# holandes22/etcd

Measured on AMD Instinct MI355X. Metric: MsgAppResp applied/sec + commits advanced/sec, 1M raft groups×3, 1-8 GPUs, higher is better.
Workload: dtype u64

## Files before the change

etcd_amd/csrc/hipbatch.hip:

```cpp
#include <hip/hip_runtime.h>

#include <algorithm>
#include <cstdio>
#include <cstdlib>
#include <cstring>
#include <type_traits>
#include <utility>
#include <vector>

#include "hbmem.h"
#include "hipbatch_kernels.h"
#include "hipbatch_fast.h"
#include "hipbatch_elect.h"
#include "hipbatch_lead.h"
#include "hipbatch_wire.h"
#include "hipbatch_wire_in.h"
#include "hipbatch_wire_out.h"
#include "hipbatch_bin.h"

using namespace hb;

#define HB_CHECK(expr)                                                       \
  do {                                                                       \
    hipError_t _e = (expr);                                                  \
// ... 1067 lines not shown
  for (uint32_t i = tid; i < RG; i += ROUTE_THREADS) {
    const uint32_t c = l_cnt[i], g = gbase + i;
    bool hand = false, elect = false, ok = true;
    if (g < G) {
      bool hib = false;
      uint64_t meta = 0;
      if (EL && c > 0) meta = a.S.meta[g];
      if (hi_on && c <= (uint32_t)KMAX) {
        const uint64_t t = a.S.term[g];
#pragma unroll
        for (uint32_t k = 0; k < (uint32_t)KMAX; ++k) {
          if (k < c) {
            const uint4 r = l_slot[k][i];
            uint64_t tm, ix;
            rec_unpack(r.x, r.y, (uint64_t)r.z | ((uint64_t)r.w << 32), a.side, &tm, &ix);
            hib |= tm > t;
          }
        }
      }
      a.cnt[g] = (uint8_t)((c < CNT_MASK ? c : CNT_MASK) | (hib ? CNT_HIGHER : 0u));
      if constexpr (EL) {
        if (c > 0) {
          const uint32_t cls = handover_class((uint32_t)meta, c, hib, a.nmax, (uint32_t)KMAX);
          elect = cls == HO_ELECT;
          hand = elect || cls == HO_APPLY;
          ok = hand || cls == HO_NONE;
          if (hand) a.resume[g] = 1u << 30;
        }
        e_c = c;
        e_hand = hand;
        e_elect = elect;
        e_meta = meta;
      } else {
#pragma unroll
        for (uint32_t k = 0; k < (uint32_t)KMAX; ++k) {
          if (k < c) {
            at32(a.slot, k * G + g) = l_slot[k][i];
            if constexpr (X) at32(a.slotx, k * G + g) = l_slotx[k][i];
          }
        }
      }
    }
    uint32_t s = c;
#pragma unroll
    for (int d = 32; d >= 1; d >>= 1) s += __shfl_xor(s, d);
    if ((tid & 63) == 0 && s) atomicAdd(&l_ptot[i >> PART_LOG], s);
    if constexpr (EL) {
      const uint64_t b = __ballot(hand), bad = __ballot(!ok);
      if ((tid & 63) == 0) {
        l_pf[i >> 5] = (uint32_t)b;
        l_pf[(i >> 5) + 1] = (uint32_t)(b >> 32);
        if (bad) atomicAnd(&l_ok[i >> PART_LOG], 0u);
      }
    }
  }
  __syncthreads();
  if (tid < NP) {
    const uint32_t part = (bk << sl) + w * NP + tid;
    if (part < a.NB) {
      const uint32_t r = atomicAdd(&a.bk_fill[bk * CTR_STRIDE], a.ev_per_msg * (l_ptot[tid] + PART * a.props_on));
      const uint64_t mo =
          (uint64_t)a.ev_per_msg * ((uint64_t)a.NB * PART + lo + ((uint64_t)bk * PART << sl) * a.props_on) + r;
      a.ev_off[2 * part + 1] = mo;
      if constexpr (EL) l_moff[tid] = mo;
    }
  }
  if constexpr (EL) {
    __syncthreads();
    const uint32_t p = __builtin_amdgcn_readfirstlane(tid >> PART_LOG);
    const uint32_t g = gbase + tid;
    const bool closed = l_ok[p] != 0;
    bool done = false;
    uint32_t st_msgs = 0, st_app = 0, st_vote = 0, st_drop = 0, st_commit = 0;
    ElectLane<EN> L;
    L.won = L.lost = L.nev = 0;
    L.committed = L.last = 0;
    uint64_t last0 = 0;
    if (closed) {
      L.S = a.S;
      L.E.chunk = a.ev + l_moff[p];
      L.E.fill = &l_efill[p];
      L.g = g;
      L.meta = e_meta;
      const bool mine = e_elect && e_c <= (uint32_t)KMAX && L.self() < L.n() && !(L.meta & M_NC);
      if (mine) {
        L.load();
        last0 = L.last;
        const uint64_t commit0 = L.committed;
        uint32_t key[KMAX];
#pragma unroll
        for (uint32_t k = 0; k < (uint32_t)KMAX; ++k) key[k] = k < e_c ? l_slot[k][tid].y : 0xFFFFFFFFu;
        const uint32_t perm = arrival_perm<(uint32_t)KMAX>(key);
        uint32_t x = 0;
#pragma nounroll
        for (; x < e_c; ++x) {
          uint32_t inf, org;
          uint64_t mterm, ix;
          slot_unpack(l_slot[(perm >> (4 * x)) & 0xF][tid], a.side, &inf, &org, &mterm, &ix);
          const uint32_t type = inf & 0xF, from = (inf >> 4) & 0xF;
          if (from >= L.n() && is_response(type)) {
            st_drop++;
            continue;
          }
          if (!L.takes(type, from, mterm)) break;
          L.step(type, from, mterm, (inf >> 8) & 1u);
          st_msgs++;
          st_app += type == HB_MSG_APP_RESP;
          st_vote += type == HB_MSG_VOTE_RESP;
        }
        if (x > 0) {
          L.store();
          if (x == e_c) {
            done = true;
          } else {
            a.resume[g] = x;
            a.commit0[g] = commit0;
          }
        }
        st_commit = done && L.committed != commit0;
      }
      flag_put<false>(&l_pf[p * FLAG_WORDS], tid & (PART - 1), done);
    }
    if (g < G && e_c > 0 && (!closed || (e_hand && !done))) {
#pragma unroll
      for (uint32_t k = 0; k < (uint32_t)KMAX; ++k)
        if (k < e_c) at32(a.slot, k * G + g) = l_slot[k][tid];
    }
    const uint32_t vals[ST_N + 1] = {st_msgs, st_app, st_vote, st_drop, st_commit, L.won, L.lost, 0,
                                     (uint32_t)(L.last - last0), L.nev};
    reduce_stats(a, l_stats, vals);
    if (tid < NP * FLAG_WORDS) {
      const uint32_t p = tid / FLAG_WORDS, j = tid % FLAG_WORDS, part = (bk << sl) + w * NP + p;
      if (part < a.NB && l_ok[p]) a.pflag[(size_t)part * FLAG_WORDS + j] = l_pf[p * FLAG_WORDS + j];
    }
    if (tid < NP) {
      const uint32_t part = (bk << sl) + w * NP + tid;
      if (part < a.NB) {
        a.lskip[part] = (uint8_t)l_ok[tid];
        if (l_ok[tid]) {
          a.ev_off[2 * part] = (uint64_t)part * PART * a.ev_per_msg;
          a.ev_counts[2 * part] = 0;
          a.ev_counts[2 * part + 1] = l_efill[tid];
          uint32_t any = 0;
#pragma unroll
          for (uint32_t j = 0; j < FLAG_WORDS; ++j) any |= l_pf[tid * FLAG_WORDS + j];
          const uint32_t xs = blockIdx.x & 7;
          if (any) a.ap_list[(size_t)xs * a.NB + atomicAdd(&a.ap_cnt[xs * CTR_STRIDE], 1u)] = part;
        }
      }
    }
  }
}

template <int NMAX, uint32_t KS, bool STEADY = false>
__device__ __forceinline__ bool fast_step(const ApplyArgs& a, FollowLane<NMAX>& L, uint32_t part, uint32_t lane,
                                          bool live, bool lead, bool leader, bool fol, uint32_t prop_raw, uint32_t cnt,
                                          uint32_t (&s_info)[KS], uint32_t (&s_orig)[KS],
                                          uint64_t (&s_term)[KS], uint64_t (&s_index)[KS],
                                          uint64_t (&s_h)[KS], uint64_t (&s_c)[KS],
                                          uint64_t moff, uint32_t* l_pfill, uint32_t* l_fill, uint32_t* l_flag,
                                          uint32_t* l_eflag, uint32_t (&vals)[ST_N + 1], uint32_t& nsteady) {
  constexpr uint32_t KMAX = KS;
  const uint32_t g = part * PART + lane;
  const uint64_t last0 = L.last, commit0 = L.committed;

  bool flagged = false;
  uint32_t resume = 0;
  uint32_t st_msgs = 0, st_drop = 0, st_app = 0;

  const uint64_t poff = (uint64_t)part * PART * a.ev_per_msg;
  if (lane == 0) a.ev_off[2 * part] = poff;
  const uint32_t prop_k = live ? prop_raw : 0u;
  if constexpr (STEADY) {
    static_assert(NMAX == 3 && KS == 2, "SteadyLane is the n = 3, two-slot lane");
    if (a.steady) {
      const bool work = live && (prop_k != 0 || cnt != 0);
      const bool idle = !work && (!lead || (!(L.mlo & (uint32_t)M_RS) && L.self() < 3));
      SteadyLane P;
      P.ok = false;
      P.evm = 0;
      if (lead && work) P.plan(L, prop_k, cnt, s_info, s_orig, s_term, s_index);
      const bool steady = lead && work && P.ok;
      if (__ballot(!(steady || idle)) == 0) {
        const uint32_t evm = steady ? P.evm : 0u;
        uint32_t tot = 0, base = 0;
#pragma unroll
        for (uint32_t j = 0; j < SteadyLane::EW_P; ++j) tot += (uint32_t)__popcll(__ballot((evm >> j) & 1u));
        if (tot && (lane & 63) == 0) base = atomicAdd(l_pfill, tot);
        base = __builtin_amdgcn_readfirstlane(base);
        uint64_t* chunk = a.ev + poff;
#pragma unroll
        for (uint32_t j = 0; j < SteadyLane::EW_P; ++j) {
          const uint64_t m = __ballot((evm >> j) & 1u);
          if ((evm >> j) & 1u) chunk[base + mbcnt64(m)] = P.word(j, lane);
          base += (uint32_t)__popcll(m);
        }
        tot = 0;
        base = 0;
#pragma unroll
        for (uint32_t j = SteadyLane::EW_P; j < SteadyLane::EW; ++j) tot += (uint32_t)__popcll(__ballot((evm >> j) & 1u));
        if (tot && (lane & 63) == 0) base = atomicAdd(l_fill, tot);
        base = __builtin_amdgcn_readfirstlane(base);
        chunk = a.ev + moff;
#pragma unroll
        for (uint32_t j = SteadyLane::EW_P; j < SteadyLane::EW; ++j) {
          const uint64_t m = __ballot((evm >> j) & 1u);
          if ((evm >> j) & 1u) chunk[base + mbcnt64(m)] = P.word(j, lane);
          base += (uint32_t)__popcll(m);
        }
        if (steady) P.commit(L);
        vals[ST_MSGS] = steady ? cnt : 0u;
        vals[ST_APPRESP] = steady ? cnt : 0u;
        vals[ST_VOTERESP] = 0;
        vals[ST_DROPPED] = 0;
        vals[ST_COMMITS] = (uint32_t)(steady && P.committed != commit0);
        vals[ST_WON] = 0;
        vals[ST_LOST] = 0;
        vals[ST_FAULTS] = 0;
        vals[ST_ENTRIES] = steady ? (uint32_t)(P.last - last0) : 0u;
        vals[ST_N] = steady ? P.nev() : 0u;
        if (a.steady_cnt && __ballot(g < a.S.G) != 0) ++nsteady;
        return false;
      }
    }
  }
  L.E.chunk = a.ev + poff;
  L.E.fill = l_pfill;
  if (prop_k) {
    if (lead && L.prop_ok(prop_k)) {
      L.arrival = 0xFFFFFFFFu;
      L.prop(prop_k);
    } else {
      flagged = true;
      resume = 1u << 31;
    }
  }

#pragma unroll
  for (uint32_t k = 0; k < KMAX; ++k) s_orig[k] = k < cnt ? s_orig[k] : 0xFFFFFFFFu;
#pragma unroll
  for (uint32_t r = 0; r < KMAX; ++r) {
#pragma unroll
    for (uint32_t k = (r & 1); k + 1 < KMAX; k += 2) {
      const bool sw = s_orig[k + 1] < s_orig[k];
      const uint32_t i0 = s_info[k], o0 = s_orig[k];
      const uint64_t t0 = s_term[k], x0 = s_index[k], h0 = s_h[k], c0 = s_c[k];
      s_info[k] = sw ? s_info[k + 1] : i0;
      s_orig[k] = sw ? s_orig[k + 1] : o0;
      s_term[k] = sw ? s_term[k + 1] : t0;
      s_index[k] = sw ? s_index[k + 1] : x0;
      s_h[k] = sw ? s_h[k + 1] : h0;
      s_c[k] = sw ? s_c[k + 1] : c0;
      s_info[k + 1] = sw ? i0 : s_info[k + 1];
      s_orig[k + 1] = sw ? o0 : s_orig[k + 1];
      s_term[k + 1] = sw ? t0 : s_term[k + 1];
      s_index[k + 1] = sw ? x0 : s_index[k + 1];
      s_h[k + 1] = sw ? h0 : s_h[k + 1];
      s_c[k + 1] = sw ? c0 : s_c[k + 1];
    }
  }
  L.E.chunk = a.ev + moff;
  L.E.fill = l_fill;
  uint32_t j = 0;
  if (live && !lead && !fol && cnt > 0 && !flagged) {
    flagged = true;
    resume = 0;
  }
  if (live && cnt > KMAX && !flagged && !L.faulted()) {
    flagged = true;
    resume = 0;
  }
  if (lead) {
#pragma unroll
    for (uint32_t k = 0; k < KMAX; ++k) {
      if (k >= cnt || flagged || L.faulted()) break;
      const uint32_t inf = s_info[k];
      const uint32_t type = inf & 0xF, from = (inf >> 4) & 0xF;
      const bool reject = (inf >> 8) & 1u;
      if (from >= L.n() && is_response(type)) {
        st_drop++;
        j++;
        continue;
      }
      if (KMAX >= 3 && type == HB_MSG_PROP) {
        if (s_term[k] != 0 || s_index[k] > 0xFFFFFFFFull || !L.prop_ok((uint32_t)s_index[k])) {
          flagged = true;
          resume = j;
          break;
        }
        L.arrival = s_orig[k];
        L.prop((uint32_t)s_index[k]);
        st_msgs++;
        j++;
        continue;
      }
      if (!L.accept_ok(type, from, s_term[k], reject)) {
        flagged = true;
        resume = j;
        break;
      }
      L.arrival = s_orig[k];
      L.accept(from, s_index[k]);
      st_msgs++;
      if (KMAX >= 3) st_app++;
      j++;
    }
  }
  bool fstepped = false;
  if (fol) {
#pragma unroll
    for (uint32_t k = 0; k < KMAX; ++k) {
      if (k >= cnt || flagged || L.faulted()) break;
      const uint32_t inf = s_info[k];
      const uint32_t from = (inf >> 4) & 0xF;
      if (!L.takes_follow(inf, from, s_term[k], s_index[k], s_h[k], s_c[k])) {
        flagged = true;
        resume = j;
        break;
      }
      L.arrival = s_orig[k];
      L.step_follow(inf, from, s_term[k], s_index[k], s_h[k], s_c[k]);
      fstepped = true;
      st_msgs++;
      j++;
    }
  }

  if (lead) L.store();
  if (fstepped) L.store_follow();
  const bool stored = lead || fstepped;
  if constexpr (NMAX >= 5) {
    bool higher = false;
#pragma unroll
    for (uint32_t k = 0; k < KMAX; ++k) higher |= k < cnt && s_term[k] > L.term;
    flag_put<true>(l_eflag, lane, flagged && (!leader || higher));
  }
  flag_put<true>(l_flag, lane, flagged);
  if (flagged) {
    at32(a.resume, g) = resume | (stored ? 0u : 1u << 30);
    if (stored) at32(a.commit0, g) = commit0;
  }
  vals[ST_MSGS] = st_msgs;
  vals[ST_APPRESP] = KMAX >= 3 ? st_app : (lead ? st_msgs : 0u);
  vals[ST_VOTERESP] = 0;
  vals[ST_DROPPED] = st_drop;
  vals[ST_COMMITS] = (uint32_t)(!flagged && L.committed != commit0);
  vals[ST_WON] = 0;
  vals[ST_LOST] = 0;
  vals[ST_FAULTS] = (uint32_t)(L.faulted() != 0 && live);
  vals[ST_ENTRIES] = (uint32_t)(L.last - last0);
  vals[ST_N] = L.nev;
  return flagged;
}

__device__ __forceinline__ void fast_close(const ApplyArgs& a, uint32_t part, const uint32_t* l_flag,
                                           const uint32_t* l_eflag, uint32_t pfill, uint32_t fill) {
  a.ev_counts[2 * part] = pfill;
  a.ev_counts[2 * part + 1] = fill;
  uint32_t any = 0, eany = 0;
#pragma unroll
  for (uint32_t w = 0; w < FLAG_WORDS; ++w) {
    any |= l_flag[w];
    eany |= l_eflag ? l_eflag[w] : 0u;
  }
  const uint32_t xs = blockIdx.x & 7;
  if (any)
    a.ap_list[(size_t)xs * a.NB + atomicAdd(&a.ap_cnt[xs * CTR_STRIDE], 1u)] = part;
  if (eany)
    a.el_list[(size_t)xs * a.NB + atomicAdd(&a.el_cnt[xs * CTR_STRIDE], 1u)] = part;
}

template <int NMAX, bool X, uint32_t KMAX>
__global__ void __launch_bounds__(PART, HB_FAST_WAVES) k_apply_fast(ApplyArgs a) {
  static_assert(NMAX <= 3, "n >= 5 leaders and followers step in k_apply_lead");
  __shared__ uint32_t l_fill, l_pfill;
  __shared__ uint32_t l_flag[FLAG_WORDS];
  __shared__ uint32_t l_eflag[FLAG_WORDS];
  __shared__ uint64_t l_stats[ST_N + 1];
  __shared__ uint32_t l_steady;

  const uint32_t part = block_part(a.sis_log);
  if (part >= a.NB) return;
  const uint32_t tid = threadIdx.x;
  const uint32_t g = part * PART + tid;
  const bool gvalid = g < a.S.G;
  if (tid == 0) l_fill = l_pfill = l_steady = 0;
  if (tid <= ST_N) l_stats[tid] = 0;
  if (tid < FLAG_WORDS) l_flag[tid] = l_eflag[tid] = 0;

  FollowLane<NMAX> L;
  L.S = a.S;
  L.g = g;
  L.mlo = gvalid ? at32(reinterpret_cast<uint32_t*>(a.S.meta), 2 * g) : 0u;
  const uint32_t prop_raw = (a.props && gvalid) ? at32(a.props, g) : 0u;
  const uint32_t cnt = gvalid ? at32(a.cnt, g) & CNT_MASK : 0u;
  if (gvalid) L.load_head();
  const bool live = gvalid && L.n() != 0 && L.faulted() == 0;
  const bool leader = live && L.state() == HB_STATE_LEADER;
  const bool nc = (L.mlo & (uint32_t)M_NC) != 0;
  const bool lead = leader && !nc && (cnt <= KMAX || prop_raw != 0);
  const bool fol = X && live && !nc && L.state() == HB_STATE_FOLLOWER && cnt > 0 && cnt <= KMAX && prop_raw == 0;
  L.dirty = 0;
  L.nev = 0;
  if (lead) {
    L.load_rest();
  } else if (fol) {
    L.load_follow();
  } else {
    L.last = L.committed = 0;
    if (!(NMAX >= 5 && leader)) L.term = 0;
  }
  uint32_t s_info[KMAX], s_orig[KMAX];
  uint64_t s_term[KMAX], s_index[KMAX], s_h[KMAX], s_c[KMAX];
  const bool slots = (lead || fol) && cnt <= KMAX;
  uint4 raw[KMAX];
#pragma unroll
  for (uint32_t k = 0; k < KMAX; ++k) {
    const bool u = NMAX >= 5 ? leader && k < cnt : slots && k < cnt;
    raw[k] = u ? at32(a.slot, k * a.S.G + g) : make_uint4(0, 0, 0, 0);
  }
#pragma unroll
  for (uint32_t k = 0; k < KMAX; ++k) slot_unpack(raw[k], a.side, &s_info[k], &s_orig[k], &s_term[k], &s_index[k]);
#pragma unroll
  for (uint32_t k = 0; k < KMAX; ++k) {
    uint4 x = make_uint4(0, 0, 0, 0);
    if (X && fol && k < cnt) x = at32(a.slotx, k * a.S.G + g);
    s_h[k] = (uint64_t)x.x | ((uint64_t)x.y << 32);
    s_c[k] = (uint64_t)x.z | ((uint64_t)x.w << 32);
  }
  uint32_t vals[ST_N + 1];
  constexpr bool STEADY = NMAX == 3 && KMAX == 2 && !X;
  uint32_t nsteady = 0;
  (void)fast_step<NMAX, KMAX, STEADY>(a, L, part, tid, live, lead, leader, fol, prop_raw, cnt, s_info, s_orig, s_term,
                                      s_index, s_h, s_c, a.ev_off[2 * part + 1], &l_pfill, &l_fill, l_flag, l_eflag, vals,
                                      nsteady);
  if (STEADY && a.steady_cnt && nsteady && (tid & 63) == 0) atomicAdd(&l_steady, nsteady);
  reduce_stats(a, l_stats, vals);
  if (STEADY && a.steady_cnt && tid == 0 && l_steady) atomicAdd(a.steady_cnt, l_steady);
  if (tid < FLAG_WORDS) a.pflag[(size_t)part * FLAG_WORDS + tid] = l_flag[tid];
  if constexpr (NMAX >= 5) {
    if (tid < FLAG_WORDS) a.eflag[(size_t)part * FLAG_WORDS + tid] = l_eflag[tid];
  }
  if (tid == 0) fast_close(a, part, l_flag, NMAX >= 5 ? l_eflag : nullptr, l_pfill, l_fill);
}

#ifndef HB_RF_UNROLL
#define HB_RF_UNROLL 4
#endif
#ifndef HB_RF_THREADS
#define HB_RF_THREADS 512
#endif
#ifndef HB_RF_RG_LOG
#define HB_RF_RG_LOG 11
#endif
#ifndef HB_RF_WAVES
#define HB_RF_WAVES 4
#endif
constexpr uint32_t RF_THREADS = HB_RF_THREADS;
constexpr uint32_t RF_UNROLL = HB_RF_UNROLL;
template <uint32_t KMAX, bool X> struct RouteFastGeom {
  static constexpr uint32_t RG_LOG = HB_RF_RG_LOG - (KMAX > 2 ? 1u : 0u) - (X ? 1u : 0u);
  static constexpr uint32_t RG = 1u << RG_LOG;
  static constexpr uint32_t NP = RG / PART;
};
template <uint32_t KMAX, bool X>
__global__ void __launch_bounds__(RF_THREADS, HB_RF_WAVES) k_route_fast(ApplyArgs a) {
  constexpr int NMAX = 3;
  using GM = RouteFastGeom<KMAX, X>;
  constexpr uint32_t RG = GM::RG, NP = GM::NP;
  const uint32_t sl = a.sis_log, W = 1u << (PART_LOG + sl - GM::RG_LOG);
  __shared__ uint32_t l_cnt[RG];
  __shared__ uint4 l_slot[KMAX][RG];
  __shared__ uint4 l_slotx[X ? KMAX : 1][X ? RG : 1];
  __shared__ uint32_t l_ptot[NP];
  __shared__ uint64_t l_moff[NP];
  __shared__ uint32_t l_fill[NP], l_pfill[NP];
  __shared__ uint32_t l_flag[NP][FLAG_WORDS];
  __shared__ uint64_t l_stats[ST_N + 1];
  const uint32_t x = blockIdx.x, q = x >> 3;
  const uint32_t bk = ((q / W) << 3) | (x & 7), w = q % W;
  if (bk >= a.NBK) return;
  const uint32_t tid = threadIdx.x;
  const uint32_t G = a.S.G;
  const uint32_t lg0 = w * RG;
  for (uint32_t i = tid; i < RG; i += RF_THREADS) l_cnt[i] = 0;
  if (tid < NP) {
    l_ptot[tid] = 0;
    l_fill[tid] = l_pfill[tid] = 0;
  }
  for (uint32_t i = tid; i < NP * FLAG_WORDS; i += RF_THREADS) (&l_flag[0][0])[i] = 0;
  if (tid <= ST_N) l_stats[tid] = 0;
  __syncthreads();
  const uint32_t lo = a.bk_off[bk], hi = a.bk_off[bk + 1];
  const uint32_t sub_lo = lg0 >> PART_LOG, sub_hi = (lg0 + RG) >> PART_LOG;
  for (uint32_t base = lo; base < hi; base += RF_THREADS * RF_UNROLL) {
    MsgRec m[RF_UNROLL];
    uint4 mx[X ? RF_UNROLL : 1];
    uint32_t sub[RF_UNROLL];
#pragma unroll
    for (uint32_t u = 0; u < RF_UNROLL; ++u) {
      const uint32_t p = base + u * RF_THREADS + tid;
      if (p < hi) m[u] = a.rec[p];
      if constexpr (X) mx[u] = p < hi ? a.recx[p] : make_uint4(0, 0, 0, 0);
      sub[u] = p < hi ? rec_sub(m[u].info) : 0xFFu;
    }
    if (w == 0) {
#pragma unroll
      for (uint32_t u = 0; u < RF_UNROLL; ++u) {
        const uint32_t p = base + u * RF_THREADS + tid;
        if (p < hi) a.key[p] = (uint8_t)sub[u];
      }
    }
#pragma unroll
    for (uint32_t u = 0; u < RF_UNROLL; ++u) {
      const uint32_t p = base + u * RF_THREADS + tid;
      const bool own = p < hi && sub[u] >= sub_lo && sub[u] < sub_hi;
      const uint32_t l = own ? (((sub[u] - sub_lo) << PART_LOG) | ((m[u].info >> 16) & (PART - 1))) : RG;
      if (l < RG) {
        const uint32_t r = atomicAdd(&l_cnt[l], 1u);
        if (r < KMAX) {
          l_slot[r][l] = make_uint4(m[u].info, m[u].orig, (uint32_t)m[u].ti, (uint32_t)(m[u].ti >> 32));
          if constexpr (X) l_slotx[r][l] = mx[X ? u : 0];
        }
      }
    }
  }
  __syncthreads();
  for (uint32_t i = tid; i < RG; i += RF_THREADS) {
    uint32_t s = l_cnt[i];
#pragma unroll
    for (int d = 32; d >= 1; d >>= 1) s += __shfl_xor(s, d);
    if ((tid & 63) == 0 && s) atomicAdd(&l_ptot[i >> PART_LOG], s);
  }
  __syncthreads();
  const uint32_t part0 = (bk << sl) + w * NP;
  if (tid < NP) {
    const uint32_t part = part0 + tid;
    uint64_t mo = 0;
    if (part < a.NB) {
      const uint32_t r = atomicAdd(&a.bk_fill[bk * CTR_STRIDE], a.ev_per_msg * (l_ptot[tid] + PART * a.props_on));
      mo = (uint64_t)a.ev_per_msg * ((uint64_t)a.NB * PART + lo + ((uint64_t)bk * PART << sl) * a.props_on) + r;
      a.ev_off[2 * part + 1] = mo;
    }
    l_moff[tid] = mo;
    l_ptot[tid] = 0;
  }
  __syncthreads();
  uint32_t acc[ST_N + 1];
#pragma unroll
  for (int k = 0; k <= ST_N; ++k) acc[k] = 0;
  constexpr bool STEADY = KMAX == 2 && !X;
  uint32_t nsteady = 0;
  for (uint32_t i = tid; i < RG; i += RF_THREADS) {
    const uint32_t p = STEADY ? (uint32_t)__builtin_amdgcn_readfirstlane(i >> PART_LOG) : i >> PART_LOG;
    const uint32_t part = part0 + p, lane = i & (PART - 1);
    const uint32_t g = part * PART + lane;
    const bool gvalid = part < a.NB && g < G;
    uint64_t moff = l_moff[p];
    if constexpr (STEADY)
      moff = (uint64_t)(uint32_t)__builtin_amdgcn_readfirstlane((uint32_t)moff) |
             (uint64_t)(uint32_t)__builtin_amdgcn_readfirstlane((uint32_t)(moff >> 32)) << 32;
    FollowLane<NMAX> L;
    L.S = a.S;
    L.g = g;
    L.mlo = gvalid ? at32(reinterpret_cast<uint32_t*>(a.S.meta), 2 * g) : 0u;
    const uint32_t prop_raw = (a.props && gvalid) ? at32(a.props, g) : 0u;
    const uint32_t c = gvalid ? l_cnt[i] : 0u;
    const uint32_t cnt = c < CNT_MASK ? c : CNT_MASK;
    if (gvalid) L.load_head();
    const bool live = gvalid && L.n() != 0 && L.faulted() == 0;
    const bool leader = live && L.state() == HB_STATE_LEADER;
    const bool nc = (L.mlo & (uint32_t)M_NC) != 0;
    const bool lead = leader && !nc && (cnt <= KMAX || prop_raw != 0);
    const bool fol = X && live && !nc && L.state() == HB_STATE_FOLLOWER && cnt > 0 && cnt <= KMAX && prop_raw == 0;
    L.dirty = 0;
    L.nev = 0;
    if (lead) {
      L.load_rest();
    } else if (fol) {
      L.load_follow();
    } else {
      L.last = L.committed = 0;
      L.term = 0;
    }
    uint32_t s_info[KMAX], s_orig[KMAX];
    uint64_t s_term[KMAX], s_index[KMAX], s_h[KMAX], s_c[KMAX];
    const bool slots = (lead || fol) && cnt <= KMAX;
#pragma unroll
    for (uint32_t k = 0; k < KMAX; ++k) {
      const bool u = slots && k < cnt;
      slot_unpack(u ? l_slot[k][i] : make_uint4(0, 0, 0, 0), a.side, &s_info[k], &s_orig[k], &s_term[k], &s_index[k]);
      uint4 xe = make_uint4(0, 0, 0, 0);
      if constexpr (X) {
        if (fol && k < cnt) xe = l_slotx[k][i];
      }
      s_h[k] = (uint64_t)xe.x | ((uint64_t)xe.y << 32);
      s_c[k] = (uint64_t)xe.z | ((uint64_t)xe.w << 32);
    }
    uint32_t vals[ST_N + 1];
    const bool flagged = fast_step<NMAX, KMAX, STEADY>(a, L, part, lane, live, lead, leader, fol, prop_raw, cnt, s_info,
                                                       s_orig, s_term, s_index, s_h, s_c, moff, &l_pfill[p],
                                                       &l_fill[p], l_flag[p], nullptr, vals, nsteady);
#pragma unroll
    for (int k = 0; k <= ST_N; ++k)
      if (!(STEADY && k == ST_APPRESP)) acc[k] += vals[k];
    if (flagged) {
      a.cnt[g] = (uint8_t)cnt;
#pragma unroll
      for (uint32_t k = 0; k < KMAX; ++k) {
        if (k < c) {
          at32(a.slot, k * G + g) = l_slot[k][i];
          if constexpr (X) at32(a.slotx, k * G + g) = l_slotx[k][i];
        }
      }
    }
  }
  if constexpr (STEADY) acc[ST_APPRESP] = acc[ST_MSGS];
  if (STEADY && a.steady_cnt && nsteady && (tid & 63) == 0) atomicAdd(&l_ptot[0], nsteady);
  reduce_stats(a, l_stats, acc);
  if (STEADY && a.steady_cnt && tid == 0 && l_ptot[0]) atomicAdd(a.steady_cnt, l_ptot[0]);
  for (uint32_t j = tid; j < NP * FLAG_WORDS; j += RF_THREADS) {
    const uint32_t p = j / FLAG_WORDS, part = part0 + p;
    if (part < a.NB) a.pflag[(size_t)part * FLAG_WORDS + j % FLAG_WORDS] = l_flag[p][j % FLAG_WORDS];
  }
  if (tid < NP && part0 + tid < a.NB) fast_close(a, part0 + tid, l_flag[tid], nullptr, l_pfill[tid], l_fill[tid]);
}

#ifndef HB_GEN_WAVES
#define HB_GEN_WAVES 2
#endif
struct GenShared {
  Stage<CHUNK> sl;
  uint32_t l_fill;
  uint32_t l_flag[FLAG_WORDS];
  uint32_t l_next[FLAG_WORDS];
  uint64_t l_stats[ST_N + 1];
};

template <int NMAX, bool FOLLOW>
__device__ __forceinline__ bool apply_part(const ApplyArgs& a, uint32_t part, GenShared& sh, bool chained) {
  const uint32_t tid = threadIdx.x;
  const uint32_t bk = part >> a.sis_log, sub = part & ((1u << a.sis_log) - 1);
  const uint32_t g = part * PART + tid;
  const uint32_t fill0 = chained ? sh.l_fill : a.ev_counts[2 * part + 1];
  if (tid < FLAG_WORDS) {
    sh.l_flag[tid] = chained ? sh.l_next[tid] : a.pflag[(size_t)part * FLAG_WORDS + tid];
    sh.l_next[tid] = 0;
  }
  __syncthreads();
  uint32_t any = 0;
#pragma unroll
  for (uint32_t w = 0; w < FLAG_WORDS; ++w) any |= sh.l_flag[w];
  if (!any) return false;
  const bool flagged = (sh.l_flag[tid >> 5] >> (tid & 31)) & 1u;

  if (tid == 0) sh.l_fill = fill0;
  if (tid <= ST_N) sh.l_stats[tid] = 0;

  Lane<NMAX, FOLLOW> L;
  L.S = a.S;
  L.E.chunk = a.ev + a.ev_off[2 * part + 1];
  L.E.fill = &sh.l_fill;
  L.g = g;
  L.won = 0;
  L.lost = 0;
  L.nev = 0;
  L.dirty = 0;
  L.prog = false;
  L.voted = false;
  L.meta = 0;
  L.last = 0;
  L.committed = 0;
  uint32_t resume = 0;
  uint64_t commit0 = 0;
  if (flagged) {
    L.meta = a.S.meta[g];
    L.load_group();
    resume = a.resume[g];
    commit0 = ((resume >> 30) & 1u) ? L.committed : a.commit0[g];
  }
  const uint64_t last0 = L.last;
  uint32_t st_msgs = 0, st_app = 0, st_vote = 0, st_drop = 0;
  const uint32_t skip = resume & 0x3FFFFFFFu;
  uint32_t j = 0;
  bool handed = false;
  uint32_t hand_at = 0;
  const uint32_t lo = a.bk_off[bk], hi = a.bk_off[bk + 1];

  constexpr uint32_t KS = route_kmax(NMAX);
  const uint32_t cnt = flagged ? a.cnt[g] & CNT_MASK : 0u;
  const bool by_slot = flagged && cnt <= a.kmax;
  const bool by_walk = flagged && !by_slot;
  __syncthreads();
  auto step_one = [&](uint32_t inf, uint32_t morig, uint64_t mterm, uint64_t mindex, uint32_t ordinal) -> bool {
    const uint32_t type = inf & 0xF, from = (inf >> 4) & 0xF;
    const bool reject = (inf >> 8) & 1u;
    if (!FOLLOW && is_follower_type(type)) {
      handed = true;
      hand_at = ordinal;
      return false;
    }
    if (from >= L.n() && is_response(type)) {
      st_drop++;
      return true;
    }
    L.arrival = morig;
    L.voted = (inf & HB_INFO_VOTED) != 0;
    const bool wants_hint = (reject && type == HB_MSG_APP_RESP) || (FOLLOW && is_follower_type(type));
    L.step(type, from, mterm, mindex, reject, (wants_hint && a.hint) ? a.hint[morig] : 0ull);
    st_msgs++;
    st_app += type == HB_MSG_APP_RESP;
    st_vote += type == HB_MSG_VOTE_RESP;
    return true;
  };
  if (by_slot) {
    if (resume >> 31) {
      L.arrival = 0xFFFFFFFFu;
      L.step(HB_MSG_PROP, L.self(), 0, a.props[g], false, 0);
    }
    uint32_t key[KS];
    uint32_t perm = 0;
#pragma unroll
    for (uint32_t k = 0; k < KS; ++k) {
      key[k] = k < cnt ? at32(a.slot, k * a.S.G + g).y : 0xFFFFFFFFu;
      perm |= k << (4 * k);
    }
#pragma unroll
    for (uint32_t r = 0; r < KS; ++r) {
#pragma unroll
      for (uint32_t k = (r & 1); k + 1 < KS; k += 2) {
        const uint32_t k0 = key[k], k1 = key[k + 1];
        const bool sw = k1 < k0;
        key[k] = sw ? k1 : k0;
        key[k + 1] = sw ? k0 : k1;
        const uint32_t p0 = (perm >> (4 * k)) & 0xF, p1 = (perm >> (4 * (k + 1))) & 0xF;
        const uint32_t swp = (perm & ~(0xFFu << (4 * k))) | (p1 << (4 * k)) | (p0 << (4 * (k + 1)));
        perm = sw ? swp : perm;
      }
    }
    uint32_t inf_n = 0, orig_n = 0;
    uint64_t term_n = 0, index_n = 0;
    if (cnt > skip)
      slot_unpack(at32(a.slot, ((perm >> (4 * skip)) & 0xF) * a.S.G + g), a.side, &inf_n, &orig_n, &term_n, &index_n);
#pragma nounroll
    for (uint32_t x = skip; x < cnt; ++x) {
      if (L.faulted()) break;
      const uint32_t inf = inf_n, morig = orig_n;
      const uint64_t mterm = term_n, mindex = index_n;
      if (x + 1 < cnt)
        slot_unpack(at32(a.slot, ((perm >> (4 * (x + 1))) & 0xF) * a.S.G + g), a.side, &inf_n, &orig_n, &term_n,
                    &index_n);
      if (!step_one(inf, morig, mterm, mindex, x)) break;
    }
  }

// ... 4159 lines not shown
```

etcd_amd/csrc/hipbatch_fast.h:

```cpp
#pragma once

#include "hipbatch_kernels.h"

namespace hb {

template <int NMAX>
struct FastLane {
  DevState S;
  EvSink E;
  uint32_t g;
  uint32_t arrival;
  uint64_t term, committed, first, last, tfirst, tlast;
  uint32_t mlo;
  uint64_t match[NMAX], next[NMAX], head[NMAX];
  uint32_t pm[NMAX];
  uint32_t dirty;
  uint32_t hv;
  static constexpr bool HEADS = NMAX <= 5;
  uint32_t nev;

  __device__ __forceinline__ uint32_t n() const { return (mlo >> 2) & 7; }
  __device__ __forceinline__ uint32_t state() const { return mlo & 3; }
  __device__ __forceinline__ uint32_t self() const { return (mlo >> 5) & 0xF; }
  __device__ __forceinline__ uint32_t faulted() const { return (mlo >> 17) & 0xF; }
// ... 289 lines not shown

  __device__ __forceinline__ void prop(uint32_t k) {
    const uint64_t old = last;
    if (sz_on(S.max_msg_size))
      sz_append(S, g, old, k, term, S.edesc + (arrival == 0xFFFFFFFFu ? S.peoff[g] : S.eoff[arrival]));
    last += k;
    if (tfirst == HB_NO_INDEX) {
      tfirst = old + 1;
      dirty |= D_TFIRST;
    }
    tlast = last;
    dirty |= D_LAST | D_TRUN;
    ev(HB_EV_LAST, 0, 0, last);
    const uint32_t sf = self();
#pragma unroll
    for (int s = 0; s < NMAX; ++s) {
      if ((uint32_t)s == sf) {
        if (match[s] < last) {
          match[s] = last;
          set_pm(s, pm[s] & ~PM_PAUSED);
        }
        if (next[s] < last + 1) next[s] = last + 1;
        dirty |= 1u << (D_SLOT0 + s);
      }
    }
    maybe_commit();
    bcast_append();
    if (faulted()) ev(HB_EV_FAULT, 0, faulted(), arrival_x());
  }

  __device__ __forceinline__ void accept(uint32_t from, uint64_t index) {
    bool updated = false, old_paused = false;
#pragma unroll
    for (int s = 0; s < NMAX; ++s) {
      if ((uint32_t)s == from) {
        old_paused = pm_count(pm[s]) == S.W;
        const uint64_t nx0 = next[s];
        if (next[s] < index + 1) next[s] = index + 1;
        if (match[s] < index) {
          match[s] = index;
          set_pm(s, pm[s] & ~PM_PAUSED);
          updated = true;
          free_to(s, index, nx0);
        }
        dirty |= 1u << (D_SLOT0 + s);
      }
    }
    if (!updated) return;
    if (maybe_commit()) {
      bcast_append();
    } else if (old_paused && !faulted()) {
#pragma unroll
      for (int s = 0; s < NMAX; ++s)
        if ((uint32_t)s == from) send_append(s);
    }
    if (faulted()) ev(HB_EV_FAULT, 0, faulted(), arrival_x());
  }
};

struct SteadyFol {
  uint64_t match, next;
  uint32_t pm;
};

struct SteadyLane {
  static constexpr uint32_t EW_P = 3, EW = 7;
  static constexpr uint32_t EVM_BCAST = 0x54, EVM_COMMIT = 0x2A;
  uint64_t last, committed, tfirst, tlast;
  uint64_t smatch, snext;
  uint32_t spm;
  SteadyFol fa, fb;
  uint32_t spm0, pa0, pb0;
  uint32_t sf, sa, sb;
  uint32_t evm;
  uint32_t ltm;
  uint32_t jfirst;
  uint64_t xfirst;
  uint32_t ring_a, ring_b;
  bool add_a, add_b, touch_a, touch_b;
  bool prop, d_tfirst;
  bool ok;

  __device__ __forceinline__ uint32_t lt_cur(uint64_t x) const { return (tfirst <= x && x <= tlast) ? 1u : 0u; }

  __device__ __forceinline__ uint64_t send(SteadyFol& f, uint32_t& ring, bool& add, bool& touch, uint32_t W,
                                           uint64_t first) {
    const uint32_t c = pm_count(f.pm);
    ok = ok && c != W && f.next >= first;
    const uint64_t x = f.next - 1;
    if (f.next <= last) {
      uint32_t idx = pm_start(f.pm) + c;
      if (idx >= W) idx -= W;
      ring = idx;
      add = true;
      f.next = last + 1;
      touch = true;
      f.pm = pm_make(HB_PR_REPLICATE, pm_paused(f.pm), pm_start(f.pm), c + 1);
    }
    ok = ok && f.next == last + 1;
    return x;
  }
  __device__ __forceinline__ void bcast(uint32_t W, uint64_t first, uint32_t j) {
    const uint64_t xa = send(fa, ring_a, add_a, touch_a, W, first);
    const uint64_t xb = send(fb, ring_b, add_b, touch_b, W, first);
    ok = ok && xa == xb;
    if (jfirst == 0) {
      jfirst = j;
      xfirst = xa;
    }
    evm |= 1u << j;
    ltm |= lt_cur(xa) << j;
  }
  __device__ __forceinline__ bool maybe_commit(uint64_t term, uint64_t first, uint32_t j) {
    const uint64_t mx = umax64(smatch, fa.match), mn = umin64(smatch, fa.match);
    const uint64_t mci = umax64(mn, umin64(mx, fb.match));
    const bool teq = (mci + 1 < first || mci > last) ? term == 0 : (tfirst <= mci && mci <= tlast);
    const bool up = mci > committed && teq;
    ok = ok && !(up && (last < mci || (evm & EVM_COMMIT) != 0));
    if (up) {
      committed = mci;
      evm |= 1u << j;
    }
    return up;
  }
  __device__ __forceinline__ void ack(uint32_t info, uint64_t mterm, uint64_t index, uint64_t term, uint32_t W,
                                      uint64_t first, uint32_t t) {
    const uint32_t type = info & 0xF, from = (info >> 4) & 0xF;
    const bool reject = (info >> 8) & 1u;
    ok = ok && type == HB_MSG_APP_RESP && !reject && (mterm == 0 || mterm == term) && (from == sa || from == sb);
    const bool isa = from == sa;
    const uint64_t am = fa.match, an = fa.next, bm = fb.match, bn = fb.next;
    const uint32_t ap = fa.pm, bp = fb.pm;
    const uint64_t m0 = isa ? am : bm, nx0 = isa ? an : bn;
    const uint32_t p0 = isa ? ap : bp;
    const uint32_t c = pm_count(p0);
    ok = ok && c != W && m0 < index && index <= last && nx0 != 0 && index >= nx0 - 1;
    const uint64_t nx = umax64(nx0, index + 1);
    uint32_t idx = pm_start(p0) + c;
    if (c != 0 && idx >= W) idx -= W;
    const uint32_t p = pm_make(HB_PR_REPLICATE, 0, idx, 0);
    fa.match = isa ? index : am;
    fa.next = isa ? nx : an;
    fa.pm = isa ? p : ap;
    touch_a = touch_a || isa;
    fb.match = isa ? bm : index;
    fb.next = isa ? bn : nx;
    fb.pm = isa ? bp : p;
    touch_b = touch_b || !isa;
    add_a = add_a && !isa;
    add_b = add_b && isa;
    if (maybe_commit(term, first, EW_P + 2 * t)) bcast(W, first, EW_P + 2 * t + 1);
  }

  __device__ __forceinline__ void plan(const FastLane<3>& L, uint32_t prop_k, uint32_t cnt,
                                       const uint32_t (&s_info)[2], const uint32_t (&s_orig)[2],
                                       const uint64_t (&s_term)[2], const uint64_t (&s_index)[2]) {
    const uint32_t W = L.S.W;
    last = L.last;
    committed = L.committed;
    tfirst = L.tfirst;
    tlast = L.tlast;
    sf = L.self();
    sa = sf == 0 ? 1u : 0u;
    sb = sf == 2 ? 1u : 2u;
    const uint64_t m0 = L.match[0], m1 = L.match[1], m2 = L.match[2];
    const uint64_t n0 = L.next[0], n1 = L.next[1], n2 = L.next[2];
    const uint32_t p0 = L.pm[0], p1 = L.pm[1], p2 = L.pm[2];
    smatch = sf == 0 ? m0 : (sf == 1 ? m1 : m2);
    snext = sf == 0 ? n0 : (sf == 1 ? n1 : n2);
    spm = spm0 = sf == 0 ? p0 : (sf == 1 ? p1 : p2);
    fa.match = sf == 0 ? m1 : m0;
    fa.next = sf == 0 ? n1 : n0;
    fa.pm = pa0 = sf == 0 ? p1 : p0;
    fb.match = sf == 2 ? m1 : m2;
    fb.next = sf == 2 ? n1 : n2;
    fb.pm = pb0 = sf == 2 ? p1 : p2;
    add_a = add_b = touch_a = touch_b = false;
    ring_a = ring_b = 0;
    evm = ltm = jfirst = 0;
    xfirst = 0;
    prop = d_tfirst = false;
    ok = L.n() == 3 && sf < 3 && !(L.mlo & (uint32_t)M_RS) && L.S.max_msg_size == HB_NO_LIMIT && cnt <= 2 &&
         pm_state(fa.pm) == HB_PR_REPLICATE && pm_state(fb.pm) == HB_PR_REPLICATE;
    if (prop_k) {
      prop = true;
      const uint64_t old = last;
      last += prop_k;
      if (tfirst == HB_NO_INDEX) {
        tfirst = old + 1;
        d_tfirst = true;
      }
      tlast = last;
      evm |= 1u;
      if (smatch < last) {
        smatch = last;
        spm &= ~PM_PAUSED;
      }
      if (snext < last + 1) snext = last + 1;
      maybe_commit(L.term, L.first, 1);
      bcast(W, L.first, 2);
    }
    const uint32_t ia = s_info[0], ib = s_info[1], oa = s_orig[0], ob = s_orig[1];
    const uint64_t ta = s_term[0], tb = s_term[1], xa = s_index[0], xb = s_index[1];
    const bool sw = cnt == 2 && ob < oa;
    const uint32_t i0 = sw ? ib : ia, i1 = sw ? ia : ib;
    const uint64_t t0 = sw ? tb : ta, t1 = sw ? ta : tb;
    const uint64_t x0 = sw ? xb : xa, x1 = sw ? xa : xb;
    if (cnt == 2) ok = ok && ((i0 ^ i1) & 0xF0u) != 0;
    if (cnt >= 1) ack(i0, t0, x0, L.term, W, L.first, 0);
    if (cnt >= 2) ack(i1, t1, x1, L.term, W, L.first, 1);
    ok = ok && ((last | xfirst) >> 40) == 0;
  }
  __device__ __forceinline__ uint32_t nev() const { return __popc(evm) + __popc(evm & EVM_BCAST); }
  __device__ __forceinline__ uint64_t word(uint32_t j, uint32_t lane) const {
    if (j == 0) return evc_word(HB_EV_LAST, 0, 0, lane, last, false);
    if ((EVM_COMMIT >> j) & 1u) return evc_word(HB_EV_COMMIT, 0, 0, lane, committed, false);
    return evc_word(EVC_BCAST, (1u << sa) | (1u << sb), (ltm >> j) & 1u, lane, j == jfirst ? xfirst : last, false);
  }

  __device__ __forceinline__ void commit(const FastLane<3>& L) const {
    const DevState& S = L.S;
    const uint32_t g = L.g;
    const bool nx0 = (L.mlo & (uint32_t)M_NX) != 0;
    const bool nx = S.lazy_next != 0 && snext == last + 1 && fa.next == last + 1 && fb.next == last + 1;
    const bool all = nx0 && !nx;
    if (nx != nx0) at32(reinterpret_cast<uint32_t*>(S.meta), 2 * g) = L.mlo ^ (uint32_t)M_NX;
    if (committed != L.committed) at32(S.commit, g) = committed;
    if (prop) {
      at32(S.last, g) = last;
      if (d_tfirst) at32(S.tfirst, g) = tfirst;
      if (!(L.mlo & (uint32_t)M_TL)) at32(S.tlast, g) = tlast;
      if (!(L.mlo & (uint32_t)M_SM)) at32(S.match, sf * S.G + g) = smatch;
    }
    if (!(L.mlo & (uint32_t)M_SM) && !nx && (prop || all)) at32(S.next, sf * S.G + g) = snext;
    if (spm != spm0) at32(S.pm, sf * S.G + g) = spm;
    if (touch_a) at32(S.match, sa * S.G + g) = fa.match;
    if (!nx && (touch_a || all)) at32(S.next, sa * S.G + g) = fa.next;
    if (fa.pm != pa0) at32(S.pm, sa * S.G + g) = fa.pm;
    if (add_a) *L.ring_at(sa, ring_a) = last;
    if (touch_b) at32(S.match, sb * S.G + g) = fb.match;
    if (!nx && (touch_b || all)) at32(S.next, sb * S.G + g) = fb.next;
    if (fb.pm != pb0) at32(S.pm, sb * S.G + g) = fb.pm;
    if (add_b) *L.ring_at(sb, ring_b) = last;
  }
};

}
```

Measured before the change: 24.97 billion.

## Add dedicated steady-state pass in route_fast with prefetched per-group head loads

Adds a separate steady pass to k_route_fast for the n=3, KMAX=2 case. It issues each group's head-state loads (meta, term, commit, first, last, tfirst, pm) at kernel start, before the routing and counting phase, and prefetches the next iteration's head while the current one is processed. This is meant to hide global memory latency behind the shared-memory routing work. Waves that are not uniformly steady or idle are recorded in a pending mask and reprocessed by the general fast_step loop, which now runs without the STEADY path. The cost is extra registers from the preloaded head, which may lower occupancy, plus duplicate loads for waves that fall back to the general path.

```diff
diff --git a/etcd_amd/csrc/hipbatch.hip b/etcd_amd/csrc/hipbatch.hip
--- a/etcd_amd/csrc/hipbatch.hip
+++ b/etcd_amd/csrc/hipbatch.hip
@@ -1243,6 +1243,48 @@
   }
 }
 
+__device__ __forceinline__ void steady_emit(const ApplyArgs& a, const SteadyLane& P, uint32_t evm, uint32_t lane,
+                                            uint64_t poff, uint64_t moff, uint32_t* l_pfill, uint32_t* l_fill) {
+  uint32_t tot = 0, base = 0;
+#pragma unroll
+  for (uint32_t j = 0; j < SteadyLane::EW_P; ++j) tot += (uint32_t)__popcll(__ballot((evm >> j) & 1u));
+  if (tot && (lane & 63) == 0) base = atomicAdd(l_pfill, tot);
+  base = __builtin_amdgcn_readfirstlane(base);
+  uint64_t* chunk = a.ev + poff;
+#pragma unroll
+  for (uint32_t j = 0; j < SteadyLane::EW_P; ++j) {
+    const uint64_t m = __ballot((evm >> j) & 1u);
+    if ((evm >> j) & 1u) chunk[base + mbcnt64(m)] = P.word(j, lane);
+    base += (uint32_t)__popcll(m);
+  }
+  tot = 0;
+  base = 0;
+#pragma unroll
+  for (uint32_t j = SteadyLane::EW_P; j < SteadyLane::EW; ++j) tot += (uint32_t)__popcll(__ballot((evm >> j) & 1u));
+  if (tot && (lane & 63) == 0) base = atomicAdd(l_fill, tot);
+  base = __builtin_amdgcn_readfirstlane(base);
+  chunk = a.ev + moff;
+#pragma unroll
+  for (uint32_t j = SteadyLane::EW_P; j < SteadyLane::EW; ++j) {
+    const uint64_t m = __ballot((evm >> j) & 1u);
+    if ((evm >> j) & 1u) chunk[base + mbcnt64(m)] = P.word(j, lane);
+    base += (uint32_t)__popcll(m);
+  }
+}
+
+struct FastRole {
+  bool live, leader, nc, lead;
+};
+__device__ __forceinline__ FastRole fast_role(uint32_t mlo, bool valid, uint32_t cnt, uint32_t prop_raw,
+                                              uint32_t kmax) {
+  FastRole r;
+  r.live = valid && ((mlo >> 2) & 7) != 0 && ((mlo >> 17) & 0xF) == 0;
+  r.leader = r.live && (mlo & 3) == HB_STATE_LEADER;
+  r.nc = (mlo & (uint32_t)M_NC) != 0;
+  r.lead = r.leader && !r.nc && (cnt <= kmax || prop_raw != 0);
+  return r;
+}
+
 template <int NMAX, uint32_t KS, bool STEADY = false>
 __device__ __forceinline__ bool fast_step(const ApplyArgs& a, FollowLane<NMAX>& L, uint32_t part, uint32_t lane,
                                           bool live, bool lead, bool leader, bool fol, uint32_t prop_raw, uint32_t cnt,
@@ -1273,32 +1315,7 @@
       if (lead && work) P.plan(L, prop_k, cnt, s_info, s_orig, s_term, s_index);
       const bool steady = lead && work && P.ok;
       if (__ballot(!(steady || idle)) == 0) {
-        const uint32_t evm = steady ? P.evm : 0u;
-        uint32_t tot = 0, base = 0;
-#pragma unroll
-        for (uint32_t j = 0; j < SteadyLane::EW_P; ++j) tot += (uint32_t)__popcll(__ballot((evm >> j) & 1u));
-        if (tot && (lane & 63) == 0) base = atomicAdd(l_pfill, tot);
-        base = __builtin_amdgcn_readfirstlane(base);
-        uint64_t* chunk = a.ev + poff;
-#pragma unroll
-        for (uint32_t j = 0; j < SteadyLane::EW_P; ++j) {
-          const uint64_t m = __ballot((evm >> j) & 1u);
-          if ((evm >> j) & 1u) chunk[base + mbcnt64(m)] = P.word(j, lane);
-          base += (uint32_t)__popcll(m);
-        }
-        tot = 0;
-        base = 0;
-#pragma unroll
-        for (uint32_t j = SteadyLane::EW_P; j < SteadyLane::EW; ++j) tot += (uint32_t)__popcll(__ballot((evm >> j) & 1u));
-        if (tot && (lane & 63) == 0) base = atomicAdd(l_fill, tot);
-        base = __builtin_amdgcn_readfirstlane(base);
-        chunk = a.ev + moff;
-#pragma unroll
-        for (uint32_t j = SteadyLane::EW_P; j < SteadyLane::EW; ++j) {
-          const uint64_t m = __ballot((evm >> j) & 1u);
-          if ((evm >> j) & 1u) chunk[base + mbcnt64(m)] = P.word(j, lane);
-          base += (uint32_t)__popcll(m);
-        }
+        steady_emit(a, P, steady ? P.evm : 0u, lane, poff, moff, l_pfill, l_fill);
         if (steady) P.commit(L);
         vals[ST_MSGS] = steady ? cnt : 0u;
         vals[ST_APPRESP] = steady ? cnt : 0u;
@@ -1486,10 +1503,8 @@
   const uint32_t prop_raw = (a.props && gvalid) ? at32(a.props, g) : 0u;
   const uint32_t cnt = gvalid ? at32(a.cnt, g) & CNT_MASK : 0u;
   if (gvalid) L.load_head();
-  const bool live = gvalid && L.n() != 0 && L.faulted() == 0;
-  const bool leader = live && L.state() == HB_STATE_LEADER;
-  const bool nc = (L.mlo & (uint32_t)M_NC) != 0;
-  const bool lead = leader && !nc && (cnt <= KMAX || prop_raw != 0);
+  const FastRole role = fast_role(L.mlo, gvalid, cnt, prop_raw, KMAX);
+  const bool live = role.live, leader = role.leader, nc = role.nc, lead = role.lead;
   const bool fol = X && live && !nc && L.state() == HB_STATE_FOLLOWER && cnt > 0 && cnt <= KMAX && prop_raw == 0;
   L.dirty = 0;
   L.nev = 0;
@@ -1554,6 +1569,79 @@
   static constexpr uint32_t RG = 1u << RG_LOG;
   static constexpr uint32_t NP = RG / PART;
 };
+struct RouteFastGroup {
+  uint32_t p, part, lane, g;
+  bool valid;
+  __device__ __forceinline__ RouteFastGroup(const ApplyArgs& a, uint32_t part0, uint32_t i) {
+    p = (uint32_t)__builtin_amdgcn_readfirstlane(i >> PART_LOG);
+    part = part0 + p;
+    lane = i & (PART - 1);
+    g = part * PART + lane;
+    valid = part < a.NB && g < a.S.G;
+  }
+};
+
+template <uint32_t RG>
+__device__ __forceinline__ uint32_t steady_pass(const ApplyArgs& a, SteadyHead H, uint32_t part0,
+                                                const uint32_t* l_cnt, const uint4 (*l_slot)[RG],
+                                                const uint64_t* l_moff, uint32_t* l_pfill, uint32_t* l_fill,
+                                                uint32_t (&acc)[ST_N + 1], uint32_t& nsteady) {
+  constexpr uint32_t NW = RG / RF_THREADS;
+  uint32_t pend = 0;
+  uint32_t msgs = 0, commits = 0, entries = 0, nev = 0;
+#pragma unroll
+  for (uint32_t k = 0; k < NW; ++k) {
+    const uint32_t i = threadIdx.x + k * RF_THREADS;
+    const RouteFastGroup R(a, part0, i);
+    SteadyIn L(a.S, R.g, H);
+    const uint32_t prop_k = H.props;
+    const uint32_t c = R.valid ? l_cnt[i] : 0u;
+    const uint32_t cnt = c < CNT_MASK ? c : CNT_MASK;
+    const FastRole role = fast_role(L.mlo, R.valid, cnt, prop_k, 2);
+    const bool live = role.live, lead = role.lead;
+    if (lead) L.load_rest();
+    uint32_t s_info[2], s_orig[2];
+    uint64_t s_term[2], s_index[2];
+#pragma unroll
+    for (uint32_t j = 0; j < 2; ++j) {
+      const bool u = lead && cnt <= 2 && j < cnt;
+      slot_unpack(u ? l_slot[j][i] : make_uint4(0, 0, 0, 0), a.side, &s_info[j], &s_orig[j], &s_term[j], &s_index[j]);
+    }
+    uint64_t moff = l_moff[R.p];
+    moff = (uint64_t)(uint32_t)__builtin_amdgcn_readfirstlane((uint32_t)moff) |
+           (uint64_t)(uint32_t)__builtin_amdgcn_readfirstlane((uint32_t)(moff >> 32)) << 32;
+    if (k + 1 < NW) {
+      const RouteFastGroup N(a, part0, i + RF_THREADS);
+      H.load(a.S, a.props, N.g, N.valid);
+    }
+    const bool work = live && (prop_k != 0 || cnt != 0);
+    const bool idle = !work && (!lead || (!(L.mlo & (uint32_t)M_RS) && L.self() < 3));
+    SteadyLane P;
+    P.ok = false;
+    P.evm = 0;
+    if (lead && work) P.plan(L, prop_k, cnt, s_info, s_orig, s_term, s_index);
+    const bool steady = lead && work && P.ok;
+    if (__ballot(!(steady || idle)) != 0) {
+      pend |= 1u << k;
+      continue;
+    }
+    const uint64_t poff = (uint64_t)R.part * PART * a.ev_per_msg;
+    if (R.lane == 0) a.ev_off[2 * R.part] = poff;
+    steady_emit(a, P, steady ? P.evm : 0u, R.lane, poff, moff, &l_pfill[R.p], &l_fill[R.p]);
+    if (steady) P.commit(L);
+    msgs += steady ? cnt : 0u;
+    commits += (uint32_t)(steady && P.committed != L.committed);
+    entries += steady ? (uint32_t)(P.last - L.last) : 0u;
+    nev += steady ? P.nev() : 0u;
+    if (a.steady_cnt && __ballot(R.g < a.S.G) != 0) ++nsteady;
+  }
+  acc[ST_MSGS] += msgs;
+  acc[ST_COMMITS] += commits;
+  acc[ST_ENTRIES] += entries;
+  acc[ST_N] += nev;
+  return (uint32_t)__builtin_amdgcn_readfirstlane(pend);
+}
+
 template <uint32_t KMAX, bool X>
 __global__ void __launch_bounds__(RF_THREADS, HB_RF_WAVES) k_route_fast(ApplyArgs a) {
   constexpr int NMAX = 3;
@@ -1574,6 +1662,15 @@
   const uint32_t tid = threadIdx.x;
   const uint32_t G = a.S.G;
   const uint32_t lg0 = w * RG;
+  const uint32_t part0 = (bk << sl) + w * NP;
+  constexpr bool STEADY = KMAX == 2 && !X;
+  SteadyHead H0 = {};
+  if constexpr (STEADY) {
+    if (a.steady) {
+      const RouteFastGroup R(a, part0, tid);
+      H0.load(a.S, a.props, R.g, R.valid);
+    }
+  }
   for (uint32_t i = tid; i < RG; i += RF_THREADS) l_cnt[i] = 0;
   if (tid < NP) {
     l_ptot[tid] = 0;
@@ -1624,7 +1721,6 @@
     if ((tid & 63) == 0 && s) atomicAdd(&l_ptot[i >> PART_LOG], s);
   }
   __syncthreads();
-  const uint32_t part0 = (bk << sl) + w * NP;
   if (tid < NP) {
     const uint32_t part = part0 + tid;
     uint64_t mo = 0;
@@ -1640,9 +1736,14 @@
   uint32_t acc[ST_N + 1];
 #pragma unroll
   for (int k = 0; k <= ST_N; ++k) acc[k] = 0;
-  constexpr bool STEADY = KMAX == 2 && !X;
   uint32_t nsteady = 0;
-  for (uint32_t i = tid; i < RG; i += RF_THREADS) {
+  uint32_t pend = (1u << (RG / RF_THREADS)) - 1;
+  if constexpr (STEADY) {
+    if (a.steady)
+      pend = steady_pass<RG>(a, H0, part0, l_cnt, l_slot, l_moff, l_pfill, l_fill, acc, nsteady);
+  }
+  for (uint32_t i = tid, kw = 0; i < RG; i += RF_THREADS, ++kw) {
+    if (STEADY && !((pend >> kw) & 1u)) continue;
     const uint32_t p = STEADY ? (uint32_t)__builtin_amdgcn_readfirstlane(i >> PART_LOG) : i >> PART_LOG;
     const uint32_t part = part0 + p, lane = i & (PART - 1);
     const uint32_t g = part * PART + lane;
@@ -1659,10 +1760,8 @@
     const uint32_t c = gvalid ? l_cnt[i] : 0u;
     const uint32_t cnt = c < CNT_MASK ? c : CNT_MASK;
     if (gvalid) L.load_head();
-    const bool live = gvalid && L.n() != 0 && L.faulted() == 0;
-    const bool leader = live && L.state() == HB_STATE_LEADER;
-    const bool nc = (L.mlo & (uint32_t)M_NC) != 0;
-    const bool lead = leader && !nc && (cnt <= KMAX || prop_raw != 0);
+    const FastRole role = fast_role(L.mlo, gvalid, cnt, prop_raw, KMAX);
+    const bool live = role.live, leader = role.leader, nc = role.nc, lead = role.lead;
     const bool fol = X && live && !nc && L.state() == HB_STATE_FOLLOWER && cnt > 0 && cnt <= KMAX && prop_raw == 0;
     L.dirty = 0;
     L.nev = 0;
@@ -1689,9 +1788,9 @@
       s_c[k] = (uint64_t)xe.z | ((uint64_t)xe.w << 32);
     }
     uint32_t vals[ST_N + 1];
-    const bool flagged = fast_step<NMAX, KMAX, STEADY>(a, L, part, lane, live, lead, leader, fol, prop_raw, cnt, s_info,
-                                                       s_orig, s_term, s_index, s_h, s_c, moff, &l_pfill[p],
-                                                       &l_fill[p], l_flag[p], nullptr, vals, nsteady);
+    const bool flagged = fast_step<NMAX, KMAX, false>(a, L, part, lane, live, lead, leader, fol, prop_raw, cnt, s_info,
+                                                      s_orig, s_term, s_index, s_h, s_c, moff, &l_pfill[p],
+                                                      &l_fill[p], l_flag[p], nullptr, vals, nsteady);
 #pragma unroll
     for (int k = 0; k <= ST_N; ++k)
       if (!(STEADY && k == ST_APPRESP)) acc[k] += vals[k];
diff --git a/etcd_amd/csrc/hipbatch_fast.h b/etcd_amd/csrc/hipbatch_fast.h
--- a/etcd_amd/csrc/hipbatch_fast.h
+++ b/etcd_amd/csrc/hipbatch_fast.h
@@ -465,7 +465,8 @@
     if (maybe_commit(term, first, EW_P + 2 * t)) bcast(W, first, EW_P + 2 * t + 1);
   }
 
-  __device__ __forceinline__ void plan(const FastLane<3>& L, uint32_t prop_k, uint32_t cnt,
+  template <class LT>
+  __device__ __forceinline__ void plan(const LT& L, uint32_t prop_k, uint32_t cnt,
                                        const uint32_t (&s_info)[2], const uint32_t (&s_orig)[2],
                                        const uint64_t (&s_term)[2], const uint64_t (&s_index)[2]) {
     const uint32_t W = L.S.W;
@@ -531,7 +532,8 @@
     return evc_word(EVC_BCAST, (1u << sa) | (1u << sb), (ltm >> j) & 1u, lane, j == jfirst ? xfirst : last, false);
   }
 
-  __device__ __forceinline__ void commit(const FastLane<3>& L) const {
+  template <class LT>
+  __device__ __forceinline__ void commit(const LT& L) const {
     const DevState& S = L.S;
     const uint32_t g = L.g;
     const bool nx0 = (L.mlo & (uint32_t)M_NX) != 0;
@@ -558,4 +560,61 @@
   }
 };
 
+struct SteadyHead {
+  uint32_t mlo, props;
+  uint64_t term, committed, first, last, tfirst;
+  uint32_t pm[3];
+
+  __device__ __forceinline__ void load(const DevState& S, const uint32_t* props_in, uint32_t g, bool valid) {
+    const uint32_t gl = valid ? g : 0u;
+    const uint32_t* pr = props_in ? props_in : S.pm;
+    const uint32_t m = at32(reinterpret_cast<const uint32_t*>(S.meta), 2 * gl);
+    const uint32_t k = at32(pr, gl);
+    const uint64_t t = at32(S.term, gl), c = at32(S.commit, gl), f = at32(S.first, gl), l = at32(S.last, gl),
+                   tf = at32(S.tfirst, gl);
+    uint32_t p[3];
+#pragma unroll
+    for (int s = 0; s < 3; ++s) p[s] = at32(S.pm, s * S.G + gl);
+    mlo = valid ? m : 0u;
+    props = (valid && props_in) ? k : 0u;
+    term = valid ? t : 0ull;
+    committed = valid ? c : 0ull;
+    first = valid ? f : 0ull;
+    last = valid ? l : 0ull;
+    tfirst = valid ? tf : 0ull;
+#pragma unroll
+    for (int s = 0; s < 3; ++s) pm[s] = valid ? p[s] : 0u;
+  }
+};
+
+struct SteadyIn {
+  const DevState& S;
+  uint32_t g;
+  uint32_t mlo;
+  uint64_t term, committed, first, last, tfirst, tlast;
+  uint64_t match[3], next[3];
+  uint32_t pm[3];
+
+  __device__ __forceinline__ SteadyIn(const DevState& S_, uint32_t g_, const SteadyHead& H)
+      : S(S_), g(g_), mlo(H.mlo), term(H.term), committed(H.committed), first(H.first), last(H.last),
+        tfirst(H.tfirst), tlast(0), match{0, 0, 0}, next{0, 0, 0}, pm{H.pm[0], H.pm[1], H.pm[2]} {}
+  __device__ __forceinline__ uint32_t n() const { return (mlo >> 2) & 7; }
+  __device__ __forceinline__ uint32_t state() const { return mlo & 3; }
+  __device__ __forceinline__ uint32_t self() const { return (mlo >> 5) & 0xF; }
+  __device__ __forceinline__ uint32_t faulted() const { return (mlo >> 17) & 0xF; }
+  __device__ __forceinline__ uint64_t* ring_at(uint32_t s, uint32_t idx) const {
+    return S.ring + ((size_t)s * S.W + idx) * S.G + g;
+  }
+  __device__ __forceinline__ void load_rest() {
+    tlast = (mlo & (uint32_t)M_TL) ? last : at32(S.tlast, g);
+    const uint32_t sf = (mlo & (uint32_t)M_SM) ? self() : 0xFFu;
+    const bool nxl = (mlo & (uint32_t)M_NX) != 0;
+#pragma unroll
+    for (int s = 0; s < 3; ++s) {
+      match[s] = ((uint32_t)s == sf) ? last : at32(S.match, s * S.G + g);
+      next[s] = ((uint32_t)s == sf || nxl) ? last + 1 : at32(S.next, s * S.G + g);
+    }
+  }
+};
+
 }
```

Result: faster. 25.46 billion, median of 6 (+2.0%).
